# Circuitscape/Circuitscape.jl

Hardware: NVIDIA H100
Metric: pair_solves_per_sec (higher is better)
Workload: dtype f64

## Files before the change

circuitscape_b200/csrc/cs_b200.cu:

```cuda
#include "../../include/cs_b200.h"

#include <cuda_runtime.h>
#include <cub/device/device_radix_sort.cuh>
#include <cub/device/device_scan.cuh>
#include <cub/device/device_select.cuh>

#include <algorithm>
#include <chrono>
#include <cmath>
#include <cstdarg>
#include <cstdio>
#include <cstdlib>
#include <cstring>
#include <limits>
#include <string>
#include <type_traits>
#include <vector>

#include "amg_host.hpp"
#include "win_host.hpp"
#include "kernels.cuh"
#include "raster_assembly.cuh"
#include "setup_device.hpp"

// ... 1241 lines not shown
    if (panel_ends(h)) {
      k_set_ctl<<<1, 1, 0, h->stream>>>(h->d_ctl, rtol, atol, imax, 40);
      k_panel_start<T, KT><<<g, NT, 0, h->stream>>>(nelem, h->pair_b ? nullptr : (const T*)h->B, (T*)h->R,
                                                    h->mixed ? (float*)h->R32 : nullptr, h->d_ctl);
      h->stats.kernel_launches += 2;
    } else {
      CK(h, cudaMemsetAsync(h->X, 0, nelem * sizeof(T), h->stream));
      CK(h, cudaMemsetAsync(h->P, 0, nelem * sizeof(T), h->stream));
      CK(h, cudaMemcpyAsync(h->R, h->B, nelem * sizeof(T), cudaMemcpyDeviceToDevice, h->stream));
      k_set_ctl<<<1, 1, 0, h->stream>>>(h->d_ctl, rtol, atol, imax, 40);
      h->stats.kernel_launches++;
      if (h->mixed) {
        k_convert<T, float><<<g, NT, 0, h->stream>>>(nelem, (const T*)h->R, (float*)h->R32);
        h->stats.kernel_launches++;
      }
    }
    launch_vcycle<T, KT>(h, false);
    mask_z<T, KT>(h);
    if (!fused) launch_update_xp2<T, KT>(h);
  }
  CK(h, cudaGetLastError());
  const int chunk = h->amg ? std::min(h->opts.check_every, 4) : h->opts.check_every;
  const bool device_loop = h->opts.use_graph == 1 && !h->profile;
  if (device_loop) {
    int rc = run_loop<T, KT>(h);
    if (rc) return rc;
  }
  for (;;) {
    CK(h, cudaMemcpyAsync(h->h_ctl, h->d_ctl, sizeof(PanelCtl), cudaMemcpyDeviceToHost, h->stream));
    CK(h, cudaStreamSynchronize(h->stream));
    if (h->profile) harvest_profile(h);
    if (device_loop) {
      GraphSlot& gs = graph_slot(h, KT);
      h->stats.kernel_launches += 1 + gs.loop_kernels * h->h_ctl->iter;
      h->stats.spmm_launches += gs.loop_spmms * h->h_ctl->iter;
      break;
    }
    if (h->h_ctl->nactive == 0) break;
    int rc = run_chunk<T, KT>(h, chunk);
    if (rc) return rc;
  }
  if (h->amg) finish_x<T, KT>(h);
  if (h->rg_on) {
    launch_spmm<T, KT, SP_RES>(h, (const T*)h->X, (T*)h->AP, (const T*)h->B);
    launch_seg_set<T, KT>(h, h->AP, 0, T(0));
    k_resnorm<T, KT><<<g, NT, 0, h->stream>>>(nelem, (size_t)h->n * KT, (const T*)h->AP, (const T*)h->B, h->d_ctl, h->d_partials);
    h->stats.kernel_launches++;
  } else {
    launch_spmm_on<T, KT, SP_RESNORM>(h, h->A0, (const T*)h->X, (T*)h->AP, (const T*)h->B, (const T*)h->d_dinv, 0.0,
                                      true, h->pair_b);
  }
  CK(h, cudaGetLastError());
  CK(h, cudaEventRecord(h->ev3, h->stream));
  CK(h, cudaMemcpyAsync(h->h_ctl, h->d_ctl, sizeof(PanelCtl), cudaMemcpyDeviceToHost, h->stream));
  CK(h, cudaStreamSynchronize(h->stream));
  if (h->profile) harvest_profile(h);
  float ms = 0;
  CK(h, cudaEventElapsedTime(&ms, h->ev2, h->ev3));
  h->stats.kernel_ms += ms;
  return CS_B200_OK;
}

int next_kt(int64_t remaining, int ktmax) {
  int kt = ktmax;
  while (kt > remaining) kt >>= 1;
  return kt < 1 ? 1 : kt;
}

#define DISPATCH_KT(kt, CALL)                    \
  switch (kt) {                                  \
    case 1: { constexpr int KT = 1; CALL; } break; \
    case 2: { constexpr int KT = 2; CALL; } break; \
    case 4: { constexpr int KT = 4; CALL; } break; \
    default: { constexpr int KT = 8; CALL; } break; \
  }

template <typename F>
decltype(auto) with_type(const cs_b200_handle* h, F&& f) {
  return h->dtype == CS_B200_F64 ? f(double{}) : f(float{});
}

template <typename F>
decltype(auto) with_width(int kt, F&& f) {
  DISPATCH_KT(kt, return f(std::integral_constant<int, KT>{}));
}

template <typename F>
decltype(auto) with_type_width(const cs_b200_handle* h, int kt, F&& f) {
  return with_type(h, [&](auto t) -> decltype(auto) {
    return with_width(kt, [&](auto KT) -> decltype(auto) { return f(t, KT); });
  });
}

struct ColumnDriver {
  cs_b200_handle* h;
  bool any_fail = false, any_maxit = false;
  std::string msg;

  template <typename Panel>
  int run(int64_t c_begin, int64_t c_end, Panel&& panel) {
    for (int64_t c0 = c_begin; c0 < c_end;) {
      const int kt = next_kt(c_end - c0, h->ktmax);
      if (int rc = with_width(kt, [&](auto KT) { return panel(KT, c0); })) return rc;
      c0 += kt;
    }
    return CS_B200_OK;
  }

  template <typename T, int KT>
  int solve(int64_t c0, double rtol, int64_t itmax, int64_t* iters, double* relres, bool masked = false) {
    h->rg_on = masked;
    const int rc = solve_panel<T, KT>(h, rtol, itmax);
    h->rg_on = false;
    h->pair_b = false;
    if (!rc) gather(KT, c0, iters, relres, itmax);
    return rc;
  }

  void gather(int kt, int64_t c0, int64_t* iters, double* relres, int64_t itmax) {
    for (int c = 0; c < kt; ++c) {
      const PanelCtl& ct = *h->h_ctl;
      const double bn = ct.bnorm[c];
      const double rr = bn > 0 ? std::sqrt(ct.resid[c] / bn) : 0.0;
      if (iters) iters[c0 + c] = ct.iters[c];
      if (relres) relres[c0 + c] = rr;
      h->stats.iterations += ct.iters[c];
      if (!(rr < h->opts.resid_gate)) {
        if (!any_fail) {
          char buf[256];
          snprintf(buf, sizeof buf,
                   "CUDA PCG solver residual %g exceeds tolerance %g for column %lld (%d iterations)",
                   rr, h->opts.resid_gate, (long long)(c0 + c + 1), ct.iters[c]);
          msg = buf;
        }
        any_fail = true;
      }
      if ((ct.iters[c] >= itmax || ct.stalled[c]) && std::sqrt(ct.rho[c]) > ct.tol[c]) any_maxit = true;
    }
  }

  int verdict(int rc) const {
    if (rc) return rc;
    if (any_fail) return set_err(h, CS_B200_ERR_RESIDUAL, "%s", msg.c_str());
    if (any_maxit) return set_err(h, CS_B200_ERR_MAXITER, "itmax reached (or the recurrence stagnated) before rtol");
    return CS_B200_OK;
  }
};

template <int KT>
int cur_grid(cs_b200_handle* h) {
  return (int)std::min<int64_t>(h->grid_spmm, (h->n + (NT / KT) - 1) / (NT / KT));
}

template <typename T, int KT>
void launch_cur_max(cs_b200_handle* h) {
  const int grid = cur_grid<KT>(h);
  if (h->A0.dia)
    k_cur_max_dia<T, KT><<<grid, NT, 0, h->stream>>>(dia_view<T>(h->A0), (const T*)h->X, h->d_ctl, h->d_partials);
  else
    k_cur_max<T, KT><<<grid, NT, 0, h->stream>>>((int)h->n, h->d_rowptr, h->d_colidx, (const T*)h->d_vals,
                                                 (const T*)h->X, h->d_ctl, h->d_partials);
  h->stats.kernel_launches++;
}

template <typename T, int KT>
void launch_currents(cs_b200_handle* h, bool want_curr, int accumulate, const void* fg = nullptr) {
  const int grid = cur_grid<KT>(h);
  launch_cur_max<T, KT>(h);
  if (h->A0.dia) {
    const DiaDev<T> a = dia_view<T>(h->A0);
    k_cur_acc_dia<T, KT><<<grid, NT, 0, h->stream>>>(a, (const T*)h->X, (const T*)fg, h->d_ctl,
                                                     want_curr ? (T*)h->AP : nullptr,
                                                     (T*)h->d_cum, (T*)h->d_max, accumulate, h->opts.log_transform, KT);
  } else {
    k_cur_acc<T, KT><<<grid, NT, 0, h->stream>>>((int)h->n, h->d_rowptr, h->d_colidx, (const T*)h->d_vals,
                                                 (const T*)h->X, (const T*)fg, h->d_ctl,
                                                 want_curr ? (T*)h->AP : nullptr,
                                                 (T*)h->d_cum, (T*)h->d_max, accumulate, h->opts.log_transform, KT);
  }
  h->stats.kernel_launches++;
}

struct ColCtl {
  long long src, dst;
  double weight;
};

inline double col_weight(const double* weight, int64_t c) { return weight ? weight[c] : 1.0; }

template <typename Col>
int upload_ctl(cs_b200_handle* h, int kt, Col&& col) {
  PanelCtl* hc = h->h_ctl;
  std::memset(hc, 0, sizeof(PanelCtl));
  for (int c = 0; c < kt; ++c) {
    const ColCtl v = col(c);
    hc->src[c] = v.src;
    hc->dst[c] = v.dst;
    hc->weight[c] = v.weight;
  }
  CK(h, cudaMemcpyAsync(h->d_ctl, hc, sizeof(PanelCtl), cudaMemcpyHostToDevice, h->stream));
  h->stats.h2d_bytes += sizeof(PanelCtl);
  return CS_B200_OK;
}

int read_ctl(cs_b200_handle* h) {
  CK(h, cudaMemcpyAsync(h->h_ctl, h->d_ctl, sizeof(PanelCtl), cudaMemcpyDeviceToHost, h->stream));
  CK(h, cudaStreamSynchronize(h->stream));
  h->stats.d2h_bytes += sizeof(PanelCtl);
  return CS_B200_OK;
}

int upload_sparse_rhs(cs_b200_handle* h, int kt, const int64_t* ptr, const int64_t* rows, const double* vals) {
  int ent_ptr[MAXKT + 1];
  for (int c = 0; c <= kt; ++c) ent_ptr[c] = (int)(ptr[c] - ptr[0]);
  const size_t nent = (size_t)ent_ptr[kt];
  if (!h->d_sp_ptr || nent > h->sp_cap) {
    cudaFree(h->d_sp_ptr); cudaFree(h->d_sp_rows); cudaFree(h->d_sp_vals);
    h->d_sp_ptr = nullptr; h->d_sp_rows = nullptr; h->d_sp_vals = nullptr;
    h->sp_cap = 0;
    const size_t cap = std::max<size_t>(nent, 1024);
    CK(h, cudaMalloc(&h->d_sp_ptr, (MAXKT + 1) * sizeof(int)));
    CK(h, cudaMalloc(&h->d_sp_rows, cap * sizeof(long long)));
    CK(h, cudaMalloc(&h->d_sp_vals, cap * sizeof(double)));
    h->sp_cap = cap;
  }
  CK(h, h2d(h, h->d_sp_ptr, ent_ptr, (kt + 1) * sizeof(int)));
  CK(h, h2d(h, h->d_sp_rows, rows + ptr[0], nent * sizeof(long long)));
  CK(h, h2d(h, h->d_sp_vals, vals + ptr[0], nent * sizeof(double)));
  h->stats.h2d_bytes += (kt + 1) * sizeof(int) + nent * 16.0;
  return CS_B200_OK;
}

int upload_set_segments(cs_b200_handle* h, int kt, const int64_t* set_ptr, const int64_t* set_rows,
                        const int64_t* set_a, const int64_t* set_b) {
  int seg[2 * MAXKT + 1];
  std::vector<int> rows;
  seg[0] = 0;
  for (int s = 0; s < 2 * kt; ++s) {
    const int64_t* sets = (s & 1) ? set_b : set_a;
    if (sets && sets[s / 2] >= 0)
      for (int64_t e = set_ptr[sets[s / 2]]; e < set_ptr[sets[s / 2] + 1]; ++e) rows.push_back((int)set_rows[e]);
    seg[s + 1] = (int)rows.size();
  }
  if (!h->d_rg_seg || rows.size() > h->rg_cap) {
    CK(h, cudaStreamSynchronize(h->stream));
    drop_graphs(h->rgraphs);
    cudaFree(h->d_rg_seg); cudaFree(h->d_rg_rows);
    h->d_rg_seg = nullptr; h->d_rg_rows = nullptr;
    h->rg_cap = 0;
    const size_t cap = std::max<size_t>(rows.size(), 4096);
    CK(h, cudaMalloc(&h->d_rg_seg, (2 * MAXKT + 1) * sizeof(int)));
    CK(h, cudaMalloc(&h->d_rg_rows, cap * sizeof(int)));
    h->rg_cap = cap;
  }
  CK(h, h2d(h, h->d_rg_seg, seg, (2 * kt + 1) * sizeof(int)));
  CK(h, h2d(h, h->d_rg_rows, rows.data(), rows.size() * sizeof(int)));
  h->stats.h2d_bytes += (2.0 * kt + 1 + rows.size()) * sizeof(int);
  return CS_B200_OK;
}

int upload_probe(cs_b200_handle* h, int64_t nprobe, const int64_t* probe) {
  const size_t need = (size_t)nprobe;
  if (need > h->probe_cap) {
    cudaFree(h->d_probe); cudaFree(h->d_probe_out);
    h->d_probe = nullptr; h->d_probe_out = nullptr;
    h->probe_cap = 0;
    CK(h, cudaMalloc(&h->d_probe, need * sizeof(long long)));
    CK(h, cudaMalloc(&h->d_probe_out, need * MAXKT * sizeof(double)));
    h->probe_cap = need;
  }
  CK(h, h2d(h, h->d_probe, probe, need * sizeof(long long)));
  return CS_B200_OK;
}

template <typename T, int KT>
int download_outputs(cs_b200_handle* h, int64_t c0, T* curr, T* volt, int volt_shift) {
  CK(h, cudaGetLastError());
  const int tg = copy_grid((size_t)h->n_pad * KT);
  auto download = [&](const void* panel, int shift, T* out) -> int {
    k_panel_to_cm<T, KT><<<tg, 256, 0, h->stream>>>((int)h->n, (size_t)h->n, (const T*)panel, (T*)h->stage,
                                                    h->d_ctl, shift);
    h->stats.kernel_launches++;
    CK(h, cudaMemcpyAsync(out + (size_t)c0 * h->n, h->stage, (size_t)h->n * KT * sizeof(T),
                          cudaMemcpyDeviceToHost, h->stream));
    h->stats.d2h_bytes += (double)h->n * KT * sizeof(T);
    return CS_B200_OK;
  };
  if (curr)
    if (int rc = download(h->AP, 0, curr)) return rc;
  if (volt)
    if (int rc = download(h->X, volt_shift, volt)) return rc;
  return CS_B200_OK;
}

template <typename T, int KT>
int currents_and_outputs(cs_b200_handle* h, int64_t c0, T* curr, T* volt, int accumulate, int volt_shift,
                         const void* fg = nullptr) {
  if (accumulate || curr) launch_currents<T, KT>(h, curr != nullptr, accumulate, fg);
  return download_outputs<T, KT>(h, c0, curr, volt, volt_shift);
}

template <typename T, int KT>
int stage_pair_rhs(cs_b200_handle* h) {
  h->pair_b = panel_ends(h);
  if (h->pair_b) return CS_B200_OK;
  CK(h, cudaMemsetAsync(h->B, 0, (size_t)h->n_pad * KT * sizeof(T), h->stream));
  k_pair_rhs<T, KT><<<1, 32, 0, h->stream>>>((T*)h->B, h->d_ctl);
  h->stats.kernel_launches++;
  return CS_B200_OK;
}

template <typename T, int KT>
int pairs_panel(cs_b200_handle* h, int64_t c0, const int64_t* src, const int64_t* dst,
                const double* weight, double rtol, int64_t itmax, T* R, T* volt, T* curr,
                int accumulate, int64_t* iters, double* relres, ColumnDriver& cols) {
  if (int rc = upload_ctl(h, KT, [&](int c) {
        return ColCtl{src[c0 + c], dst[c0 + c], col_weight(weight, c0 + c)};
      }))
    return rc;
  if (int rc = stage_pair_rhs<T, KT>(h)) return rc;
  if (int rc = cols.solve<T, KT>(c0, rtol, itmax, iters, relres)) return rc;
  k_pair_extract<T, KT><<<1, 32, 0, h->stream>>>((const T*)h->X, h->d_ctl);
// ... 1963 lines not shown
```

circuitscape_b200/csrc/kernels.cuh:

```cuda
#pragma once
#include <cuda_runtime.h>
#include <stdint.h>

namespace csb {

constexpr int NT = 256;
constexpr int NWARP = NT / 32;
constexpr int NNZ_CAP = 2304;
constexpr int MAXKT = 8;

struct PanelCtl {
  double rho[MAXKT];
  double pap[MAXKT];
  double alpha[MAXKT];
  double beta[MAXKT];
  double tol[MAXKT];
  double rho0[MAXKT];
  double resid[MAXKT];
  double bnorm[MAXKT];
  double xsrc[MAXKT];
  double xdst[MAXKT];
  double maxpos[MAXKT];
  double maxneg[MAXKT];
  double weight[MAXKT];
// ... 2140 lines not shown
__global__ void __launch_bounds__(NT)
k_panel_start(size_t nelem, const T* __restrict__ B, T* __restrict__ R, float* __restrict__ R32,
              const PanelCtl* __restrict__ ctl) {
  constexpr int VEC = Vec<T>::N;
  const size_t stride = (size_t)gridDim.x * NT * VEC;
  for (size_t e = ((size_t)blockIdx.x * NT + threadIdx.x) * VEC; e < nelem; e += stride) {
    T r[VEC];
    if (B) {
      vload(B + e, r);
    } else {
#pragma unroll
      for (int i = 0; i < VEC; ++i) r[i] = pair_rhs_at<T, KT>(ctl, e + i);
    }
    vstore(R + e, r);
    if (R32) {
      if constexpr (VEC == 2)
        *reinterpret_cast<float2*>(R32 + e) = make_float2((float)r[0], (float)r[1]);
      else
        *reinterpret_cast<float4*>(R32 + e) = make_float4((float)r[0], (float)r[1], (float)r[2], (float)r[3]);
    }
  }
}

template <typename T, int KT>
__global__ void __launch_bounds__(NT)
k_jacobi0(size_t nelem, const T* __restrict__ B, const T* __restrict__ dinv, T omega,
          T* __restrict__ X) {
  constexpr int VEC = Vec<T>::N;
  constexpr int L = Log2<KT>::v;
  const size_t stride = (size_t)gridDim.x * NT * VEC;
  for (size_t e = ((size_t)blockIdx.x * NT + threadIdx.x) * VEC; e < nelem; e += stride) {
    T b[VEC], x[VEC];
    vload(B + e, b);
#pragma unroll
    for (int i = 0; i < VEC; ++i) x[i] = omega * dinv[(e + i) >> L] * b[i];
    vstore(X + e, x);
  }
}

template <typename T, int KT>
__global__ void __launch_bounds__(NT)
k_coarse_dense(int n, const double* __restrict__ pinv, const T* __restrict__ B, T* __restrict__ X) {
  const int e = blockIdx.x * NT + threadIdx.x;
  if (e >= n * KT) return;
  const int i = e / KT, c = e % KT;
  const double* row = pinv + (size_t)i * n;
  double a0 = 0.0, a1 = 0.0, a2 = 0.0, a3 = 0.0;
  int j = 0;
  for (; j + 3 < n; j += 4) {
    a0 += row[j] * (double)B[(size_t)j * KT + c];
    a1 += row[j + 1] * (double)B[(size_t)(j + 1) * KT + c];
    a2 += row[j + 2] * (double)B[(size_t)(j + 2) * KT + c];
    a3 += row[j + 3] * (double)B[(size_t)(j + 3) * KT + c];
  }
  for (; j < n; ++j) a0 += row[j] * (double)B[(size_t)j * KT + c];
  X[e] = (T)((a0 + a1) + (a2 + a3));
}

__global__ void k_loop_cond(cudaGraphConditionalHandle handle, const PanelCtl* __restrict__ ctl) {
  cudaGraphSetConditional(handle, (ctl->nactive > 0 && ctl->iter < ctl->itmax) ? 1u : 0u);
}

template <typename T>
__global__ void k_dinv(int n, int n_pad, const int* __restrict__ rowptr,
                       const int* __restrict__ colidx, const T* __restrict__ vals, T* dinv) {
  for (int i = blockIdx.x * blockDim.x + threadIdx.x; i < n_pad; i += gridDim.x * blockDim.x) {
    T d = T(0);
    if (i < n)
      for (int j = rowptr[i]; j < rowptr[i + 1]; ++j)
        if (colidx[j] == i) d += vals[j];
    dinv[i] = d != T(0) ? T(1) / d : T(0);
  }
}

template <typename T, int KT>
__global__ void k_pair_rhs(T* B, const PanelCtl* ctl) {
  const int c = threadIdx.x;
  if (c < KT) {
    const long long s = ctl->src[c], d = ctl->dst[c];
    if (s >= 0 && d >= 0 && s != d) {
      B[(size_t)s * KT + c] = T(-1);
      B[(size_t)d * KT + c] = T(1);
    }
  }
}

template <typename T, int KT>
__global__ void k_pair_extract(const T* X, PanelCtl* ctl) {
  const int c = threadIdx.x;
  if (c < KT) {
    const long long s = ctl->src[c], d = ctl->dst[c];
    ctl->xsrc[c] = s >= 0 ? (double)X[(size_t)s * KT + c] : 0.0;
    ctl->xdst[c] = d >= 0 ? (double)X[(size_t)d * KT + c] : 0.0;
  }
}

template <typename T, int KT>
__global__ void k_sparse_rhs(T* B, const int* __restrict__ ent_ptr, const long long* __restrict__ rows,
                             const double* __restrict__ vals) {
  const int c = threadIdx.x;
  if (c < KT)
    for (int e = ent_ptr[c]; e < ent_ptr[c + 1]; ++e) B[(size_t)rows[e] * KT + c] += (T)vals[e];
}

template <typename T, int KT>
__global__ void k_probe(const T* __restrict__ X, const PanelCtl* __restrict__ ctl,
                        const long long* __restrict__ probe, int nprobe, T* __restrict__ out) {
  for (int e = blockIdx.x * blockDim.x + threadIdx.x; e < nprobe * KT; e += gridDim.x * blockDim.x) {
    const int c = e / nprobe, i = e % nprobe;
    out[e] = (T)((double)X[(size_t)probe[i] * KT + c] - ctl->xsrc[c]);
  }
}

template <typename T, int KT>
__global__ void k_combine(int n, size_t n_pad, const T* __restrict__ U, const int* __restrict__ ci,
                          const int* __restrict__ cj, T* __restrict__ X) {
  const size_t total = n_pad * KT;
  for (size_t e = (size_t)blockIdx.x * blockDim.x + threadIdx.x; e < total; e += (size_t)gridDim.x * blockDim.x) {
    const size_t i = e / KT;
    const int c = (int)(e % KT);
    T v = T(0);
    if (i < (size_t)n) {
      const int a = ci[c], b = cj[c];
      v = (b >= 0 ? U[(size_t)b * n_pad + i] : T(0)) - (a >= 0 ? U[(size_t)a * n_pad + i] : T(0));
    }
    X[e] = v;
  }
}

template <typename T, int KT>
__global__ void k_cm_to_panel(int n, size_t ld, const T* __restrict__ cm, T* __restrict__ panel,
                              int ncols) {
  const size_t total = (size_t)n * KT;
  for (size_t e = (size_t)blockIdx.x * blockDim.x + threadIdx.x; e < total;
       e += (size_t)gridDim.x * blockDim.x) {
    const size_t i = e / KT;
    const int c = (int)(e % KT);
    panel[e] = c < ncols ? cm[(size_t)c * ld + i] : T(0);
  }
}
template <typename T, int KT>
__global__ void k_panel_to_cm(int n, size_t ld, const T* __restrict__ panel, T* __restrict__ cm,
                              const PanelCtl* ctl, int use_shift) {
  const size_t total = (size_t)n * KT;
  for (size_t e = (size_t)blockIdx.x * blockDim.x + threadIdx.x; e < total;
       e += (size_t)gridDim.x * blockDim.x) {
    const size_t i = e / KT;
    const int c = (int)(e % KT);
    const T sh = use_shift ? (T)ctl->xsrc[c] : T(0);
    cm[(size_t)c * ld + i] = panel[e] - sh;
  }
}

template <typename T>
__device__ __forceinline__ void ground_current(T x, T& inflow, T& outflow) {
  if (x < T(0)) inflow -= x;
  if (x > T(0)) outflow += x;
}

template <typename T, int KT>
__global__ void __launch_bounds__(NT)
k_cur_max(int n, const int* __restrict__ rowptr, const int* __restrict__ colidx,
          const T* __restrict__ vals, const T* __restrict__ V, PanelCtl* ctl, double* partials) {
  CSB_REDUCE_SMEM(2, KT)
  const int c = threadIdx.x % KT;
  constexpr int RPP = NT / KT;
  double mp = -1.0e300, mn = -1.0e300;
  for (int row = blockIdx.x * RPP + threadIdx.x / KT; row < n; row += gridDim.x * RPP) {
    const T vi = V[(size_t)row * KT + c];
    for (int j = rowptr[row]; j < rowptr[row + 1]; ++j) {
      const int col = colidx[j];
      if (col > row) {
        const T d = fabs(vals[j]) * (vi - V[(size_t)col * KT + c]);
        mp = fmax(mp, (double)d);
        mn = fmax(mn, (double)(-d));
      }
    }
  }
  double v[2][1] = {{mp}, {mn}};
  if (grid_reduce<KT, 1, 2, true>(v, partials, &ctl->ticket, s_warp, s_tree, s_out)) {
    if (threadIdx.x < KT) {
      ctl->maxpos[threadIdx.x] = s_out[threadIdx.x];
      ctl->maxneg[threadIdx.x] = s_out[KT + threadIdx.x];
    }
  }
}

template <typename T, int KT>
__global__ void __launch_bounds__(NT)
k_cur_acc(int n, const int* __restrict__ rowptr, const int* __restrict__ colidx,
          const T* __restrict__ vals, const T* __restrict__ V, const T* __restrict__ fg, const PanelCtl* ctl,
          T* __restrict__ cur_out , T* __restrict__ cum, T* __restrict__ mx,
          int accumulate, int log_transform, int ncols) {
  const int c = threadIdx.x % KT;
  constexpr int RPP = NT / KT;
  const T maxpos = (T)ctl->maxpos[c], maxneg = (T)ctl->maxneg[c];
  const double w = ctl->weight[c];
  const int nrow_iter = (n + RPP - 1) / RPP;
  for (int it = blockIdx.x; it < nrow_iter; it += gridDim.x) {
    const int row = it * RPP + threadIdx.x / KT;
    T cur = T(0);
    if (row < n) {
      const T vi = V[(size_t)row * KT + c];
      T inflow = T(0), outflow = T(0);
      for (int j = rowptr[row]; j < rowptr[row + 1]; ++j) {
        const int col = colidx[j];
        if (col == row) continue;
        const T d = fabs(vals[j]) * (vi - V[(size_t)col * KT + c]);
        if (!(fabs(d / maxneg) < T(1e-8)) && d > T(0)) outflow += d;
        if (!(fabs(d / maxpos) < T(1e-8)) && d < T(0)) inflow -= d;
      }
      if (fg) ground_current(fg[row] * vi, inflow, outflow);
      cur = inflow > outflow ? inflow : outflow;
      if (cur_out) cur_out[(size_t)row * KT + c] = cur;
    }
    if (accumulate) {
      T val = cur;
      if (log_transform) val = cur > T(0) ? (T)log10((double)cur) : T(-9999);
      const unsigned mask = 0xffffffffu;
      const int lane = threadIdx.x & 31;
      const int base = lane - c;
      double s = 0.0;
      T m = T(-1.0e30);
#pragma unroll
      for (int cc = 0; cc < KT; ++cc) {
        const T vv = __shfl_sync(mask, val, base + cc);
        const double ww = __shfl_sync(mask, w, base + cc);
        if (cc < ncols && ww != 0.0) {
          s += ww * (double)vv;
          m = vv > m ? vv : m;
        }
      }
      if (c == 0 && row < n) {
        cum[row] = (T)((double)cum[row] + s);
        if (mx) mx[row] = m > mx[row] ? m : mx[row];
      }
    }
  }
}

template <typename T, int KT>
__global__ void __launch_bounds__(NT)
k_cur_max_dia(const DiaDev<T> A, const T* __restrict__ V, PanelCtl* ctl, double* partials) {
  CSB_REDUCE_SMEM(2, KT)
  const int c = threadIdx.x % KT;
  constexpr int RPP = NT / KT;
  const int n = A.n, nr = A.nr;
  double mp = -1.0e300, mn = -1.0e300;
  for (int row = blockIdx.x * RPP + threadIdx.x / KT; row < n; row += gridDim.x * RPP) {
    T a[4], vj[4];
    const T vi = V[(size_t)row * KT + c];
#pragma unroll
    for (int q = 0; q < 4; ++q) {
      const int s = 5 + q;
      a[q] = __ldg(A.run(s) + row);
      const int j = min(n - 1, row + (s / 3 - 1) * nr + (s % 3 - 1));
      vj[q] = V[(size_t)j * KT + c];
    }
#pragma unroll
    for (int q = 0; q < 4; ++q)
      if (a[q] != T(0)) {
        const T d = fabs(a[q]) * (vi - vj[q]);
        mp = fmax(mp, (double)d);
        mn = fmax(mn, (double)(-d));
      }
  }
  double v[2][1] = {{mp}, {mn}};
  if (grid_reduce<KT, 1, 2, true>(v, partials, &ctl->ticket, s_warp, s_tree, s_out)) {
    if (threadIdx.x < KT) {
      ctl->maxpos[threadIdx.x] = s_out[threadIdx.x];
      ctl->maxneg[threadIdx.x] = s_out[KT + threadIdx.x];
    }
  }
}

template <typename T, int KT>
__global__ void __launch_bounds__(NT)
k_cur_acc_dia(const DiaDev<T> A, const T* __restrict__ V, const T* __restrict__ fg, const PanelCtl* ctl,
              T* __restrict__ cur_out,
              T* __restrict__ cum, T* __restrict__ mx, int accumulate, int log_transform, int ncols) {
  const int c = threadIdx.x % KT;
  constexpr int RPP = NT / KT;
  const int n = A.n, nr = A.nr;
  const T maxpos = (T)ctl->maxpos[c], maxneg = (T)ctl->maxneg[c];
  const double w = ctl->weight[c];
  const int nrow_iter = (n + RPP - 1) / RPP;
  for (int it = blockIdx.x; it < nrow_iter; it += gridDim.x) {
    const int row = it * RPP + threadIdx.x / KT;
    T cur = T(0);
    if (row < n) {
      T a[9], vj[9];
#pragma unroll
      for (int s = 0; s < 9; ++s) {
        a[s] = A.at(s, row);
        const int j = max(0, min(n - 1, row + (s / 3 - 1) * nr + (s % 3 - 1)));
        vj[s] = V[(size_t)j * KT + c];
      }
      const T vi = vj[4];
      T inflow = T(0), outflow = T(0);
#pragma unroll
      for (int s = 0; s < 9; ++s) {
        if (s == 4) continue;
        const T d = fabs(a[s]) * (vi - vj[s]);
        if (!(fabs(d / maxneg) < T(1e-8)) && d > T(0)) outflow += d;
        if (!(fabs(d / maxpos) < T(1e-8)) && d < T(0)) inflow -= d;
      }
      if (fg) ground_current(fg[row] * vi, inflow, outflow);
      cur = inflow > outflow ? inflow : outflow;
      if (cur_out) cur_out[(size_t)row * KT + c] = cur;
    }
    if (accumulate) {
      T val = cur;
      if (log_transform) val = cur > T(0) ? (T)log10((double)cur) : T(-9999);
      const unsigned mask = 0xffffffffu;
      const int lane = threadIdx.x & 31;
      const int base = lane - c;
      double s = 0.0;
      T m = T(-1.0e30);
#pragma unroll
      for (int cc = 0; cc < KT; ++cc) {
        const T vv = __shfl_sync(mask, val, base + cc);
        const double ww = __shfl_sync(mask, w, base + cc);
        if (cc < ncols && ww != 0.0) {
          s += ww * (double)vv;
          m = vv > m ? vv : m;
        }
      }
      if (c == 0 && row < n) {
        cum[row] = (T)((double)cum[row] + s);
        if (mx) mx[row] = m > mx[row] ? m : mx[row];
      }
    }
  }
}

__global__ void k_branch_count(int n, const int* __restrict__ rowptr, const int* __restrict__ colidx,
                               int* __restrict__ cnt, int* bad_row) {
  for (int row = blockIdx.x * blockDim.x + threadIdx.x; row < n; row += gridDim.x * blockDim.x) {
    int low = 0;
    for (int j = rowptr[row]; j < rowptr[row + 1]; ++j) {
      const int col = colidx[j];
      if (j > rowptr[row] && col <= colidx[j - 1]) atomicMin(bad_row, row);
      low += col < row;
    }
    cnt[row] = low;
  }
}

__global__ void k_branch_ends(int n, const int* __restrict__ rowptr, const int* __restrict__ colidx,
                              const int* __restrict__ bptr, long long* __restrict__ lo, long long* __restrict__ hi) {
  for (int row = blockIdx.x * blockDim.x + threadIdx.x; row < n; row += gridDim.x * blockDim.x)
    for (int e = bptr[row], j = rowptr[row]; e < bptr[row + 1]; ++e, ++j) {
      lo[e] = colidx[j];
      hi[e] = row;
    }
}

template <typename T, int KT>
__global__ void __launch_bounds__(NT)
k_branch_cur(int n, const int* __restrict__ rowptr, const int* __restrict__ colidx, const T* __restrict__ vals,
             const int* __restrict__ bptr, const T* __restrict__ V, const PanelCtl* ctl, T* __restrict__ out,
             size_t ld, T* __restrict__ cum, int ncols) {
  T maxpos[KT];
#pragma unroll
  for (int c = 0; c < KT; ++c) maxpos[c] = (T)ctl->maxpos[c];
  for (int row = blockIdx.x * NT + threadIdx.x; row < n; row += gridDim.x * NT) {
    const int e0 = bptr[row], e1 = bptr[row + 1];
    if (e0 == e1) continue;
    T vhi[KT];
#pragma unroll
    for (int c = 0; c < KT; ++c) vhi[c] = V[(size_t)row * KT + c];
    for (int e = e0, j = rowptr[row]; e < e1; ++e, ++j) {
      const int lo = colidx[j];
      const T a = fabs(vals[j]);
      double s = 0.0;
#pragma unroll
      for (int c = 0; c < KT; ++c) {
        const T d = a * (V[(size_t)lo * KT + c] - vhi[c]);
        const T b = !(fabs(d / maxpos[c]) < T(1e-8)) ? fabs(d) : T(0);
        if (out) out[(size_t)c * ld + e] = b;
        if (cum) {
          const double w = ctl->weight[c];
          if (c < ncols && w != 0.0) s += w * (double)b;
        }
      }
      if (cum) cum[e] = (T)((double)cum[e] + s);
    }
  }
}

template <typename T, int KT>
__global__ void k_owner_sum(int n, const T* __restrict__ X, const long long* __restrict__ owner, long long c0,
                            T* __restrict__ vsum) {
  for (int row = blockIdx.x * blockDim.x + threadIdx.x; row < n; row += gridDim.x * blockDim.x) {
    const long long c = owner[row] - c0;
    if (c >= 0 && c < KT) vsum[row] += X[(size_t)row * KT + c];
  }
}

__global__ void k_set_ctl(PanelCtl* ctl, double rtol, double atol, int itmax, int stall_limit) {
  ctl->stall_limit = stall_limit;
  ctl->rtol = rtol;
  ctl->atol = atol;
  ctl->itmax = itmax;
  ctl->init = 1;
  ctl->iter = 0;
}

__global__ void k_set_stall(PanelCtl* ctl, int stall_limit) { ctl->stall_limit = stall_limit; }

template <typename T>
__global__ void k_fill(T* p, size_t n, T v) {
  for (size_t i = (size_t)blockIdx.x * blockDim.x + threadIdx.x; i < n;
       i += (size_t)gridDim.x * blockDim.x)
    p[i] = v;
}

__global__ void k_flush(float* p, size_t n) {
  for (size_t i = (size_t)blockIdx.x * blockDim.x + threadIdx.x; i < n;
       i += (size_t)gridDim.x * blockDim.x)
    p[i] = p[i] * 1.0001f + 1.0f;
}

template <typename T, int KT>
__global__ void __launch_bounds__(NT)
k_seg_set(T* __restrict__ P, const int* __restrict__ seg, const int* __restrict__ rows, int set_b_only, T v) {
  const int s = blockIdx.x;
  if (set_b_only && !(s & 1)) return;
  const int c = s >> 1;
  for (int e = seg[s] + threadIdx.x; e < seg[s + 1]; e += NT) P[(size_t)rows[e] * KT + c] = v;
}

template <typename T, int KT>
__global__ void __launch_bounds__(NT)
k_seg_current(T* __restrict__ C, const int* __restrict__ seg, const int* __restrict__ rows) {
  __shared__ double s_sum[NT];
  const int s = blockIdx.x, c = s >> 1, tid = threadIdx.x;
  double a = 0.0;
  for (int e = seg[s] + tid; e < seg[s + 1]; e += NT) a += (double)C[(size_t)rows[e] * KT + c];
  s_sum[tid] = a;
  __syncthreads();
  for (int w = NT / 2; w > 0; w >>= 1) {
    if (tid < w) s_sum[tid] += s_sum[tid + w];
    __syncthreads();
  }
  const T tot = (T)s_sum[0];
  for (int e = seg[s] + tid; e < seg[s + 1]; e += NT) C[(size_t)rows[e] * KT + c] = tot;
}

template <typename T, int KT>
__global__ void __launch_bounds__(NT)
k_resnorm(size_t nelem, size_t nvalid, const T* __restrict__ Y, const T* __restrict__ B, PanelCtl* ctl,
          double* partials) {
  constexpr int VEC = Vec<T>::N;
  CSB_REDUCE_SMEM(2, KT)
  const size_t stride = (size_t)gridDim.x * NT * VEC;
  double acc[2][VEC];
#pragma unroll
  for (int i = 0; i < VEC; ++i) acc[0][i] = acc[1][i] = 0.0;
  for (size_t e = ((size_t)blockIdx.x * NT + threadIdx.x) * VEC; e < nelem; e += stride) {
    T y[VEC], b[VEC];
    vload(Y + e, y);
    vload(B + e, b);
#pragma unroll
    for (int i = 0; i < VEC; ++i) {
      if (e + i >= nvalid) continue;
      acc[0][i] += (double)y[i] * (double)y[i];
      acc[1][i] += (double)b[i] * (double)b[i];
    }
  }
  if (grid_reduce<KT, VEC, 2, false>(acc, partials, &ctl->ticket, s_warp, s_tree, s_out)) {
    if (threadIdx.x < KT) {
      ctl->resid[threadIdx.x] = s_out[threadIdx.x];
      ctl->bnorm[threadIdx.x] = s_out[KT + threadIdx.x];
    }
  }
}

template <typename T, int KT>
__global__ void __launch_bounds__(NT)
k_flux(size_t nelem, size_t nvalid, const T* __restrict__ U, const T* __restrict__ AU, PanelCtl* ctl,
       double* partials) {
  constexpr int VEC = Vec<T>::N;
  CSB_REDUCE_SMEM(1, KT)
  const size_t stride = (size_t)gridDim.x * NT * VEC;
  double acc[1][VEC];
// ... 289 lines not shown
```

profiles/run_panel_ends.py:

```python
#!/usr/bin/env python
import argparse
import json
import os
import re
import subprocess
import sys
import tempfile
from collections import defaultdict

ROOT = os.path.dirname(os.path.dirname(os.path.abspath(__file__)))
sys.path.insert(0, ROOT)
SWITCH = "CS_B200_NO_FUSED_PANEL_ENDS"


def card():
    try:
        out = subprocess.run(["nvidia-smi", "--query-gpu=name,power.limit", "--format=csv,noheader"],
                             capture_output=True, text=True, timeout=30).stdout.strip().splitlines()
        name, pl = [s.strip() for s in out[0].split(",")]
        return {"name": name, "power_limit": pl}
    except Exception as e:
        return {"name": None, "power_limit": None, "error": str(e)}


def short(name):
    name = name.replace("(anonymous namespace)::", "").replace("csb::", "")
    name = re.sub(r"^void ", "", name)
    depth, cut = 0, len(name)
    for i, ch in enumerate(name):
        if ch == "<":
            depth += 1
        elif ch == ">":
            depth -= 1
        elif ch == "(" and depth == 0 and i > 0:
            cut = i
            break
    return name[:cut].replace(" ", "")


def child(rows, npairs, trace_path):
    import numpy as np
    import torch
    from torch.profiler import ProfilerActivity, profile
    import circuitscape_b200 as cb
    from circuitscape_b200 import graph

    L, _ = graph.synthetic_raster_laplacian(rows, rows, seed=42)
    npts = 2
    while npts * (npts - 1) // 2 < 128:
        npts += 1
    src, dst = graph.all_pairs(graph.focal_nodes(L.shape[0], npts, seed=7), limit=128)
    src, dst = src[:npairs], dst[:npairs]
    with cb.construct_cholesky_factor(L, cb.CUDASolver()) as f:
        f.reset_currents()
        f.solve_pairs(src, dst, accumulate=True)
        torch.cuda.synchronize()
        f.reset_currents()
        with profile(activities=[ProfilerActivity.CUDA]) as prof:
            out = f.solve_pairs(src, dst, accumulate=True)
            torch.cuda.synchronize()
        prof.export_chrome_trace(trace_path)
        np.save(trace_path + ".R.npy", np.asarray(out["R"]))


def panels(trace_path):
    with open(trace_path) as fh:
        ev = json.load(fh)["traceEvents"]
    dev = sorted((e for e in ev if e.get("ph") == "X" and e.get("cat") in ("kernel", "gpu_memset", "gpu_memcpy")),
                 key=lambda e: e["ts"])
    out, cur = [], []
    for e in dev:
        cur.append(e)
        if short(e["name"]).startswith("k_cur_acc_dia"):
            out.append(cur)
            cur = []
    res = []
    for p in out:
        conds = [i for i, e in enumerate(p) if short(e["name"]).startswith("k_loop_cond")]
        if not conds:
            raise SystemExit("no k_loop_cond in a panel: the device WHILE loop did not run")
        start, end = p[:conds[0]], p[conds[-1] + 1:]

        def passes(seg):
            agg = defaultdict(lambda: [0, 0.0])
            for e in seg:
                k = short(e["name"])
                agg[k][0] += 1
                agg[k][1] += e["dur"] / 1000.0
            return [{"pass": k, "launches": n, "ms": round(ms, 4)} for k, (n, ms) in agg.items()]

        res.append({"start_ms": round(sum(e["dur"] for e in start) / 1000.0, 4),
                    "end_ms": round(sum(e["dur"] for e in end) / 1000.0, 4),
                    "loop_cond_kernels": len(conds),
                    "start": passes(start), "end": passes(end)})
    return res


def main():
    ap = argparse.ArgumentParser()
    ap.add_argument("--rows", type=int, default=3163)
    ap.add_argument("--pairs", type=int, default=16)
    ap.add_argument("--out", default=None)
    ap.add_argument("--child", default=None, help=argparse.SUPPRESS)
    a = ap.parse_args()
    if a.child:
        child(a.rows, a.pairs, a.child)
        return
    import numpy as np
    result = {"card": card(), "rows": a.rows, "pairs": a.pairs, "settings": {}}
    with tempfile.TemporaryDirectory() as tmp:
        R = {}
        for name, off in (("on", False), ("off", True)):
            env = dict(os.environ)
            env.pop(SWITCH, None)
            if off:
                env[SWITCH] = "1"
            trace = os.path.join(tmp, f"{name}.json")
            subprocess.run([sys.executable, os.path.abspath(__file__), "--rows", str(a.rows), "--pairs", str(a.pairs),
                            "--child", trace], env=env, check=True, cwd=ROOT)
            ps = panels(trace)
            R[name] = np.load(trace + ".R.npy")
            result["settings"][name] = {
                "start_ms_per_panel": round(sum(p["start_ms"] for p in ps) / len(ps), 4),
                "end_ms_per_panel": round(sum(p["end_ms"] for p in ps) / len(ps), 4),
                "panels": ps}
        result["R_identical"] = bool(np.array_equal(R["on"], R["off"]))
    line = json.dumps(result)
    print(line)
    if a.out:
        with open(a.out, "w") as fh:
            fh.write(line + "\n")


if __name__ == "__main__":
    main()
```

Baseline: 147.8.

## Add cp.async stencil-pipelined current max/accumulate kernels for DIA matrices

```diff
diff --git a/circuitscape_b200/csrc/cs_b200.cu b/circuitscape_b200/csrc/cs_b200.cu
--- a/circuitscape_b200/csrc/cs_b200.cu
+++ b/circuitscape_b200/csrc/cs_b200.cu
@@ -1417,10 +1417,31 @@
   return (int)std::min<int64_t>(h->grid_spmm, (h->n + (NT / KT) - 1) / (NT / KT));
 }
 
+inline bool cur_pipe(const cs_b200_handle* h) {
+  static const bool off = std::getenv("CS_B200_NO_CUR_PIPE") != nullptr;
+  return !off && h->A0.dia && stencil_pipe();
+}
+
+template <typename T, int KT, bool HALF>
+void launch_cur_acc_pipe(cs_b200_handle* h, const DiaDev<T>& a, const T* fg, T* cur_out, int accumulate) {
+  using CP = CurPipe<T, KT, HALF>;
+  constexpr int SMEM = CP::DAcc::BYTES;
+  set_max_smem_once<k_cur_acc_pipe<T, KT, HALF>>(h, SMEM);
+  const int grid = wave_grid(h, k_cur_acc_pipe<T, KT, HALF>, SMEM, h->A0, CP::RPP);
+  k_cur_acc_pipe<T, KT, HALF><<<grid, NT, SMEM, h->stream>>>(a, (const T*)h->X, fg, h->d_ctl, cur_out, (T*)h->d_cum,
+                                                             (T*)h->d_max, accumulate, h->opts.log_transform, KT);
+}
+
 template <typename T, int KT>
 void launch_cur_max(cs_b200_handle* h) {
   const int grid = cur_grid<KT>(h);
-  if (h->A0.dia)
+  if (cur_pipe(h)) {
+    using CP = CurPipe<T, KT, false>;
+    constexpr int SMEM = CP::DMax::BYTES;
+    set_max_smem_once<k_cur_max_pipe<T, KT>>(h, SMEM);
+    const int wg = wave_grid(h, k_cur_max_pipe<T, KT>, SMEM, h->A0, CP::RPP);
+    k_cur_max_pipe<T, KT><<<wg, NT, SMEM, h->stream>>>(dia_view<T>(h->A0), (const T*)h->X, h->d_ctl, h->d_partials);
+  } else if (h->A0.dia)
     k_cur_max_dia<T, KT><<<grid, NT, 0, h->stream>>>(dia_view<T>(h->A0), (const T*)h->X, h->d_ctl, h->d_partials);
   else
     k_cur_max<T, KT><<<grid, NT, 0, h->stream>>>((int)h->n, h->d_rowptr, h->d_colidx, (const T*)h->d_vals,
@@ -1432,7 +1453,12 @@
 void launch_currents(cs_b200_handle* h, bool want_curr, int accumulate, const void* fg = nullptr) {
   const int grid = cur_grid<KT>(h);
   launch_cur_max<T, KT>(h);
-  if (h->A0.dia) {
+  if (cur_pipe(h)) {
+    const DiaDev<T> a = dia_view<T>(h->A0);
+    T* const cur_out = want_curr ? (T*)h->AP : nullptr;
+    if (a.half) launch_cur_acc_pipe<T, KT, true>(h, a, (const T*)fg, cur_out, accumulate);
+    else launch_cur_acc_pipe<T, KT, false>(h, a, (const T*)fg, cur_out, accumulate);
+  } else if (h->A0.dia) {
     const DiaDev<T> a = dia_view<T>(h->A0);
     k_cur_acc_dia<T, KT><<<grid, NT, 0, h->stream>>>(a, (const T*)h->X, (const T*)fg, h->d_ctl,
                                                      want_curr ? (T*)h->AP : nullptr,
diff --git a/circuitscape_b200/csrc/kernels.cuh b/circuitscape_b200/csrc/kernels.cuh
--- a/circuitscape_b200/csrc/kernels.cuh
+++ b/circuitscape_b200/csrc/kernels.cuh
@@ -2316,6 +2316,30 @@
   }
 }
 
+template <typename T> struct CutConst;
+template <> struct CutConst<double> {
+  static constexpr double T8 = 1e-8, HI = 1e-8 * (1.0 + 0x1p-50), LO = 1e-8 * (1.0 - 0x1p-50);
+  static constexpr double MIN = 0x1p-960, MAX = 0x1p960;
+};
+template <> struct CutConst<float> {
+  static constexpr float T8 = 1e-8f, HI = 1e-8f * (1.0f + 0x1p-21f), LO = 1e-8f * (1.0f - 0x1p-21f);
+  static constexpr float MIN = 0x1p-120f, MAX = 0x1p120f;
+};
+
+template <typename T>
+__host__ __device__ __forceinline__ T cut_recip(T m) {
+  const T a = fabs(m);
+  return a >= CutConst<T>::MIN && a <= CutConst<T>::MAX ? T(1) / a : T(NAN);
+}
+
+template <typename T>
+__host__ __device__ __forceinline__ bool cut_keeps(T d, T m, T r) {
+  const T q = fabs(d) * r;
+  if (q > CutConst<T>::HI) return true;
+  if (q < CutConst<T>::LO) return false;
+  return !(fabs(d / m) < CutConst<T>::T8);
+}
+
 template <typename T>
 __device__ __forceinline__ void ground_current(T x, T& inflow, T& outflow) {
   if (x < T(0)) inflow -= x;
@@ -2496,6 +2520,228 @@
       }
     }
   }
+}
+
+template <typename T, int KT, bool HALF> struct CurPipe {
+  static constexpr int V16 = 16 / (int)sizeof(T);
+  static constexpr int CPT = KT < V16 ? KT : V16;
+  static constexpr int CG = KT / CPT;
+  static constexpr int RPP = NT / CG;
+  static constexpr int PX = st_a16((RPP + 2) * KT * (int)sizeof(T));
+  static constexpr int MAX_OWN = st_a16(4 * RPP * (int)sizeof(T));
+  using DMax = StDepth<PX, MAX_OWN, 3>;
+  static constexpr int PDG = PX;
+  static constexpr int ACC_PANEL = PX + (HALF ? st_a16(5 * (RPP + 2) * (int)sizeof(T)) : 0);
+  static constexpr int OD = HALF ? 0 : st_a16(9 * RPP * (int)sizeof(T));
+  static constexpr int OR = st_a16(RPP * (int)sizeof(T));
+  static constexpr int ACC_OWN = OD + 3 * OR;
+  using DAcc = StDepth<ACC_PANEL, ACC_OWN, 3>;
+};
+
+template <typename T, int RPP, int S0, int NS>
+__device__ __forceinline__ void cp_runs(T* dst, const DiaDev<T>& A, long long row0) {
+  constexpr int NCH = NS * RPP;
+#pragma unroll 1
+  for (int q0 = 0; q0 < NCH; q0 += NT) {
+    const int q = q0 + (int)threadIdx.x;
+    if (NCH % NT == 0 || q < NCH) {
+      const long long g = row0 + q % RPP;
+      const bool ok = g < A.n;
+      cp_async_zfill<(int)sizeof(T)>(dst + q, A.run(S0 + q / RPP) + (ok ? g : 0), ok);
+    }
+  }
+}
+
+template <typename T, int KT>
+__global__ void __launch_bounds__(NT, 3)
+k_cur_max_pipe(const DiaDev<T> A, const T* __restrict__ V, PanelCtl* ctl, double* partials) {
+  using CP = CurPipe<T, KT, false>;
+  constexpr int CPT = CP::CPT, RPP = CP::RPP, S = CP::DMax::S;
+  constexpr int RP = S + 3;
+  extern __shared__ __align__(128) unsigned char st_sm[];
+  unsigned char* const pring = st_sm;
+  unsigned char* const oring = st_sm + RP * CP::PX;
+  const int tid = threadIdx.x;
+  const int cg = tid % CP::CG, rl = tid / CP::CG, c0 = cg * CPT;
+  const int n = A.n, nr = A.nr;
+  double mp[CPT], mn[CPT];
+#pragma unroll
+  for (int i = 0; i < CPT; ++i) mp[i] = mn[i] = -1.0e300;
+
+  auto issue = [&](const StStep& s, int lp, int lo) {
+    if (s.c >= s.cs) cp_rows<T, KT, RPP + 2>(reinterpret_cast<T*>(pring + lp * CP::PX), V, (long long)s.c * nr + s.r0 - 1, n);
+    if (s.c > s.cs)
+      cp_runs<T, RPP, 5, 4>(reinterpret_cast<T*>(oring + lo * CP::MAX_OWN), A, (long long)(s.c - 1) * nr + s.r0);
+  };
+  auto compute = [&](const StStep& s, int sp, int so) {
+    const int c = s.c - 1, r = s.r0 + rl;
+    if (r >= nr || (long long)c * nr + r >= n) return;
+    const T* xs[2];
+#pragma unroll
+    for (int d = 0; d < 2; ++d) {
+      const int k = sp + d + RP - 1;
+      xs[d] = reinterpret_cast<const T*>(pring + (k >= RP ? k - RP : k) * CP::PX);
+    }
+    const T* dg = reinterpret_cast<const T*>(oring + so * CP::MAX_OWN);
+    T vi[CPT];
+    ldvec<T, CPT>(xs[0] + (rl + 1) * KT + c0, vi);
+#pragma unroll
+    for (int q = 0; q < 4; ++q) {
+      const int s9 = 5 + q;
+      const T a = dg[q * RPP + rl];
+      if (a != T(0)) {
+        T vj[CPT];
+        ldvec<T, CPT>(xs[s9 / 3 - 1] + (rl + s9 % 3) * KT + c0, vj);
+#pragma unroll
+        for (int i = 0; i < CPT; ++i) {
+          const T d = fabs(a) * (vi[i] - vj[i]);
+          mp[i] = fmax(mp[i], (double)d);
+          mn[i] = fmax(mn[i], (double)(-d));
+        }
+      }
+    }
+  };
+  stencil_pipe<S, RPP>(n, nr, issue, compute);
+
+  CSB_REDUCE_SMEM(2, KT)
+  double v[2][CPT];
+#pragma unroll
+  for (int i = 0; i < CPT; ++i) { v[0][i] = mp[i]; v[1][i] = mn[i]; }
+  if (grid_reduce<KT, CPT, 2, true>(v, partials, &ctl->ticket, s_warp, s_tree, s_out)) {
+    if (tid < KT) {
+      ctl->maxpos[tid] = s_out[tid];
+      ctl->maxneg[tid] = s_out[KT + tid];
+    }
+  }
+}
+
+template <typename T, int KT, bool HALF>
+__global__ void __launch_bounds__(NT, 3)
+k_cur_acc_pipe(const DiaDev<T> A, const T* __restrict__ V, const T* __restrict__ fg, const PanelCtl* ctl,
+               T* __restrict__ cur_out, T* __restrict__ cum, T* __restrict__ mx, int accumulate, int log_transform,
+               int ncols) {
+  using CP = CurPipe<T, KT, HALF>;
+  constexpr int CPT = CP::CPT, CG = CP::CG, RPP = CP::RPP, S = CP::DAcc::S;
+  constexpr int RP = S + 3;
+  extern __shared__ __align__(128) unsigned char st_sm[];
+  __shared__ double s_w[KT];
+  __shared__ T s_max[2][KT];
+  unsigned char* const pring = st_sm;
+  unsigned char* const oring = st_sm + RP * CP::ACC_PANEL;
+  const int tid = threadIdx.x;
+  const int cg = tid % CG, rl = tid / CG, c0 = cg * CPT;
+  const int n = A.n, nr = A.nr;
+  T rpos[CPT], rneg[CPT];
+#pragma unroll
+  for (int i = 0; i < CPT; ++i) {
+    rpos[i] = cut_recip((T)ctl->maxpos[c0 + i]);
+    rneg[i] = cut_recip((T)ctl->maxneg[c0 + i]);
+  }
+  if (tid < KT) {
+    s_w[tid] = ctl->weight[tid];
+    s_max[0][tid] = (T)ctl->maxpos[tid];
+    s_max[1][tid] = (T)ctl->maxneg[tid];
+  }
+  __syncthreads();
+
+  auto issue = [&](const StStep& s, int lp, int lo) {
+    unsigned char* ps = pring + lp * CP::ACC_PANEL;
+    const long long g0 = (long long)s.c * nr + s.r0 - 1;
+    cp_rows<T, KT, RPP + 2>(reinterpret_cast<T*>(ps), V, g0, n);
+    if (HALF) {
+      const int u0 = s.c >= s.cs ? 1 : 2, u1 = s.c < s.ce ? 5 : u0;
+      cp_diag_half<T, RPP>(reinterpret_cast<T*>(ps + CP::PDG), A, g0, u0, u1);
+    }
+    if (s.c > s.cs) {
+      T* os = reinterpret_cast<T*>(oring + lo * CP::ACC_OWN);
+      const long long row0 = (long long)(s.c - 1) * nr + s.r0;
+      if (!HALF) {
+        cp_runs<T, RPP, 0, 4>(os, A, row0);
+        cp_runs<T, RPP, 5, 4>(os + 5 * RPP, A, row0);
+      }
+      T* rows = reinterpret_cast<T*>(oring + lo * CP::ACC_OWN + CP::OD);
+      if (accumulate) cp_rows<T, 1, RPP>(rows, cum, row0, n);
+      if (accumulate && mx) cp_rows<T, 1, RPP>(rows + CP::OR / (int)sizeof(T), mx, row0, n);
+      if (fg) cp_rows<T, 1, RPP>(rows + 2 * CP::OR / (int)sizeof(T), fg, row0, n);
+    }
+  };
+  auto compute = [&](const StStep& s, int sp, int so) {
+    const int c = s.c - 1, r = s.r0 + rl;
+    const long long row_l = (long long)c * nr + r;
+    const bool live = r < nr && row_l < n;
+    const int row = (int)row_l;
+    const T* rows = reinterpret_cast<const T*>(oring + so * CP::ACC_OWN + CP::OD);
+    T cur[CPT];
+#pragma unroll
+    for (int i = 0; i < CPT; ++i) cur[i] = T(0);
+    if (live) {
+      const T* xs[3];
+      const T* ds[3];
+#pragma unroll
+      for (int d = 0; d < 3; ++d) {
+        const int k = sp + d + RP - 2;
+        const unsigned char* p = pring + (k >= RP ? k - RP : k) * CP::ACC_PANEL;
+        xs[d] = reinterpret_cast<const T*>(p);
+        ds[d] = reinterpret_cast<const T*>(p + CP::PDG);
+      }
+      const T* dg = reinterpret_cast<const T*>(oring + so * CP::ACC_OWN);
+      T vi[CPT], inflow[CPT], outflow[CPT];
+      ldvec<T, CPT>(xs[1] + (rl + 1) * KT + c0, vi);
+#pragma unroll
+      for (int i = 0; i < CPT; ++i) inflow[i] = outflow[i] = T(0);
+#pragma unroll
+      for (int s9 = 0; s9 < 9; ++s9) {
+        if (s9 == 4) continue;
+        T vj[CPT];
+        ldvec<T, CPT>(xs[s9 / 3] + (rl + s9 % 3) * KT + c0, vj);
+        const T a = HALF ? st_half_val<T, RPP>(ds, s9, rl) : dg[s9 * RPP + rl];
+#pragma unroll
+        for (int i = 0; i < CPT; ++i) {
+          const T d = fabs(a) * (vi[i] - vj[i]);
+          if (d > T(0) && cut_keeps(d, s_max[1][c0 + i], rneg[i])) outflow[i] += d;
+          if (d < T(0) && cut_keeps(d, s_max[0][c0 + i], rpos[i])) inflow[i] -= d;
+        }
+      }
+      const T fgv = fg ? rows[2 * CP::OR / (int)sizeof(T) + rl] : T(0);
+#pragma unroll
+      for (int i = 0; i < CPT; ++i) {
+        if (fg) ground_current(fgv * vi[i], inflow[i], outflow[i]);
+        cur[i] = inflow[i] > outflow[i] ? inflow[i] : outflow[i];
+      }
+      if (cur_out) stvec<T, CPT>(cur_out + (size_t)row * KT + c0, cur);
+    }
+    if (accumulate) {
+      T val[CPT];
+#pragma unroll
+      for (int i = 0; i < CPT; ++i) {
+        val[i] = cur[i];
+        if (log_transform) val[i] = cur[i] > T(0) ? (T)log10((double)cur[i]) : T(-9999);
+      }
+      const int base = (tid & 31) - cg;
+      double sum = 0.0;
+      T m = T(-1.0e30);
+#pragma unroll
+      for (int g = 0; g < CG; ++g)
+#pragma unroll
+        for (int i = 0; i < CPT; ++i) {
+          const int cc = g * CPT + i;
+          const T vv = CG > 1 ? __shfl_sync(0xffffffffu, val[i], base + g) : val[i];
+          const double ww = s_w[cc];
+          if (cc < ncols && ww != 0.0) {
+            sum += ww * (double)vv;
+            m = vv > m ? vv : m;
+          }
+        }
+      if (cg == 0 && live) {
+        cum[row] = (T)((double)rows[rl] + sum);
+        if (mx) {
+          const T mo = rows[CP::OR / (int)sizeof(T) + rl];
+          mx[row] = m > mo ? m : mo;
+        }
+      }
+    }
+  };
+  stencil_pipe<S, RPP>(n, nr, issue, compute);
 }
 
 __global__ void k_branch_count(int n, const int* __restrict__ rowptr, const int* __restrict__ colidx,
diff --git a/profiles/run_panel_ends.py b/profiles/run_panel_ends.py
--- a/profiles/run_panel_ends.py
+++ b/profiles/run_panel_ends.py
@@ -10,7 +10,16 @@
 
 ROOT = os.path.dirname(os.path.dirname(os.path.abspath(__file__)))
 sys.path.insert(0, ROOT)
-SWITCH = "CS_B200_NO_FUSED_PANEL_ENDS"
+HBM_PEAK = 3.35e12
+
+
+def cur_bytes(name, n):
+    m = re.match(r"k_cur_(max|acc)_(?:pipe|dia)<(double|float),(\d+)", name)
+    if not m:
+        return None
+    t = 8 if m.group(2) == "double" else 4
+    row = int(m.group(3)) * t + 4 * t + (4 * t if m.group(1) == "acc" else 0)
+    return n * row
 
 
 def card():
@@ -63,7 +72,7 @@
         np.save(trace_path + ".R.npy", np.asarray(out["R"]))
 
 
-def panels(trace_path):
+def panels(trace_path, n):
     with open(trace_path) as fh:
         ev = json.load(fh)["traceEvents"]
     dev = sorted((e for e in ev if e.get("ph") == "X" and e.get("cat") in ("kernel", "gpu_memset", "gpu_memcpy")),
@@ -71,7 +80,7 @@
     out, cur = [], []
     for e in dev:
         cur.append(e)
-        if short(e["name"]).startswith("k_cur_acc_dia"):
+        if re.match(r"k_cur_acc_(dia|pipe)<", short(e["name"])):
             out.append(cur)
             cur = []
     res = []
@@ -89,10 +98,18 @@
                 agg[k][1] += e["dur"] / 1000.0
             return [{"pass": k, "launches": n, "ms": round(ms, 4)} for k, (n, ms) in agg.items()]
 
+        currents = []
+        for e in end:
+            b = cur_bytes(short(e["name"]), n)
+            if b:
+                s = e["dur"] / 1e6
+                currents.append({"pass": short(e["name"]), "ms": round(e["dur"] / 1000.0, 4), "GB": round(b / 1e9, 4),
+                                 "GB_per_s": round(b / s / 1e9, 1), "of_hbm_peak": round(b / s / HBM_PEAK, 3)})
         res.append({"start_ms": round(sum(e["dur"] for e in start) / 1000.0, 4),
                     "end_ms": round(sum(e["dur"] for e in end) / 1000.0, 4),
+                    "currents_ms": round(sum(c["ms"] for c in currents), 4),
                     "loop_cond_kernels": len(conds),
-                    "start": passes(start), "end": passes(end)})
+                    "start": passes(start), "end": passes(end), "currents": currents})
     return res
 
 
@@ -100,6 +117,8 @@
     ap = argparse.ArgumentParser()
     ap.add_argument("--rows", type=int, default=3163)
     ap.add_argument("--pairs", type=int, default=16)
+    ap.add_argument("--switch", default="CS_B200_NO_FUSED_PANEL_ENDS",
+                    help="environment variable that turns the change off (set in the 'off' run)")
     ap.add_argument("--out", default=None)
     ap.add_argument("--child", default=None, help=argparse.SUPPRESS)
     a = ap.parse_args()
@@ -107,22 +126,23 @@
         child(a.rows, a.pairs, a.child)
         return
     import numpy as np
-    result = {"card": card(), "rows": a.rows, "pairs": a.pairs, "settings": {}}
+    result = {"card": card(), "rows": a.rows, "pairs": a.pairs, "switch": a.switch, "settings": {}}
     with tempfile.TemporaryDirectory() as tmp:
         R = {}
         for name, off in (("on", False), ("off", True)):
             env = dict(os.environ)
-            env.pop(SWITCH, None)
+            env.pop(a.switch, None)
             if off:
-                env[SWITCH] = "1"
+                env[a.switch] = "1"
             trace = os.path.join(tmp, f"{name}.json")
             subprocess.run([sys.executable, os.path.abspath(__file__), "--rows", str(a.rows), "--pairs", str(a.pairs),
                             "--child", trace], env=env, check=True, cwd=ROOT)
-            ps = panels(trace)
+            ps = panels(trace, a.rows * a.rows)
             R[name] = np.load(trace + ".R.npy")
             result["settings"][name] = {
                 "start_ms_per_panel": round(sum(p["start_ms"] for p in ps) / len(ps), 4),
                 "end_ms_per_panel": round(sum(p["end_ms"] for p in ps) / len(ps), 4),
+                "currents_ms_per_panel": round(sum(p["currents_ms"] for p in ps) / len(ps), 4),
                 "panels": ps}
         result["R_identical"] = bool(np.array_equal(R["on"], R["off"]))
     line = json.dumps(result)
```

Measured after the change: 151.0 (median of 6 runs). 1.02x the previous value.
